# g1n0st/drake

Hardware: AMD Instinct MI355X
Metric: mpm_substeps_per_sec_1M_particles (higher is better)
Workload: dtype f32

## Files before the change

### drake_amd/csrc/mpm_step.h

```cpp
#pragma once
#include "mpm_device.h"

namespace mpm {

MPM_DEV bool gated_out(const DP& p) {
    return ((p.gated & 1) && p.ctl->need_rebuild) || ((p.gated & 2) && (p.ctl->error & ERR_SLABS)) ||
           ((p.gated & 4) && (int)(p.ctl->watch_hit - p.watch_base) >= 0);
}

template <int FM>
__global__ __launch_bounds__(256) void k_fem(DP p, float dt) {
#define MPM_FEM_MATERIAL_SETUP
#define MPM_FEM_M p.M
#define MPM_FEM_VOLW p.dist.on ? S.q[0][i].w : f2.w
#include "mpm_fem_face.inc"
#undef MPM_FEM_MATERIAL_SETUP
#undef MPM_FEM_M
#undef MPM_FEM_VOLW
}

struct ClothMat {
    float mu, lambda, gamma, K, cF, rho, pad0, pad1;
};
constexpr int FACE_CLOTH_SHIFT = 12;
MPM_DEV Material cloth_material(const Material& engine, const ClothMat* mats, const float4& f3) {
    const ClothMat t = mats[(unsigned)__float_as_int(f3.x) >> FACE_CLOTH_SHIFT];
    Material m = engine;
    m.mu = t.mu; m.lambda = t.lambda; m.gamma = t.gamma; m.K = t.K; m.cF = t.cF; m.density = t.rho;
    return m;
}

template <int FM>
__global__ __launch_bounds__(256) void k_fem_mat(DP p, float dt, const ClothMat* mats) {
#define MPM_FEM_MATERIAL_SETUP const Material M = cloth_material(p.M, mats, f3);
#define MPM_FEM_M M
#define MPM_FEM_VOLW f2.w * M.density
#include "mpm_fem_face.inc"
#undef MPM_FEM_MATERIAL_SETUP
#undef MPM_FEM_M
#undef MPM_FEM_VOLW
}

MPM_DEV bool vertex_force_vf(const DP& p, int k, float& f0, float& f1, float& f2) {
    const float* e0 = p.VF + vf_entry((unsigned)k, 0) * 3;
    float3 g[8];
#pragma unroll
    for (int j = 0; j < 8; ++j) g[j] = *reinterpret_cast<const float3*>(e0 + (size_t)j * VF_CHUNK * 3);
    f0 = f1 = f2 = 0.f;
#pragma unroll
    for (int j = 0; j < 8; ++j) {
        f0 += -g[j].x;
        f1 += -g[j].y;
        f2 += -g[j].z;
    }
    return __float_as_uint(g[0].x) != VF_MARK;
}

MPM_DEV void vertex_force_csr(const DP& p, const PSet& S, int k, float& f0, float& f1, float& f2) {
    const int s = p.Nf + k;
    f0 = f1 = f2 = 0.f;
    const int vo = S.pid[s] - p.NfG;
    for (int e = p.adj_off[vo]; e < p.adj_off[vo + 1]; ++e) {
        const int fc = p.adj_fc[e];
        const int fs = p.imap[fc >> 2];
        const float3 g = fs >= 0 ? p.G3[(size_t)fs * 3 + (fc & 3)]
                                 : make_float3(S.q[0][s].w > 0.f ? __int_as_float(0x7FC00000) : 0.f, 0.f, 0.f);
        f0 += -g.x;
        f1 += -g.y;
        f2 += -g.z;
    }
}

MPM_DEV void vertex_force_value(const DP& p, const PSet& S, int k, float& f0, float& f1, float& f2) {
    if (!vertex_force_vf(p, k, f0, f1, f2)) vertex_force_csr(p, S, k, f0, f1, f2);
}
MPM_DEV void vertex_force(const DP& p, const PSet& S, int k) {
    float f0, f1, f2;
    vertex_force_value(p, S, k, f0, f1, f2);
    const int s = p.Nf + k;
    p.f[0][s] = f0;
    p.f[1][s] = f1;
    p.f[2][s] = f2;
}

__global__ __launch_bounds__(256) void k_vforce(DP p) {
    if (gated_out(p)) return;
    const unsigned nva = (unsigned)p.ctl->nva;
    const unsigned chunk = xcd_chunk_active(blockIdx.x, nva);
    const int k = (int)(chunk * 256 + threadIdx.x);
    if (chunk == 0xFFFFFFFFu || k >= (int)nva) return;
    vertex_force(p, p.set[p.ctl->cur], k);
}

typedef float f32x4 __attribute__((ext_vector_type(4)));
typedef float f32x2 __attribute__((ext_vector_type(2)));

constexpr int STG = 16, STG_FX = 13;

MPM_DEV void lds_add_fixed(long long* a, float q, unsigned& worst) {
    const float aq = fabsf(q);
    const float h = floorf(aq * 0x1p-32f);
    const unsigned lo = (unsigned)rintf(fmaf(-h, 0x1p32f, aq));
    const unsigned long long mag = ((unsigned long long)(unsigned)h << 32) | lo;
    const unsigned long long fx = q < 0.f ? 0ull - mag : mag;
    __hip_atomic_fetch_add(reinterpret_cast<unsigned long long*>(a), fx, __ATOMIC_RELAXED,
                           __HIP_MEMORY_SCOPE_WORKGROUP);
    worst = max(worst, __float_as_uint(aq));
}

MPM_DEV void bspline_coeff(int a, bool on, float& c0, float& c1, float& c2) {
    c0 = a == 0 ? 1.125f : (a == 1 ? -.25f : .125f);
    c1 = a == 0 ? -1.5f : (a == 1 ? 2.f : -.5f);
    c2 = a == 1 ? -1.f : .5f;
    if (!on) c0 = c1 = c2 = 0.f;
}

struct Stencil {
    int rx, ry, rz;
    float fx[3];
    float wx[3], wy[3], wz[3];
    unsigned out_bits;
};

MPM_DEV Stencil make_stencil(const DP& p, float x, float y, float z, int ox, int oy, int oz) {
    Stencil s;
    const uint32_t hi = (uint32_t)((1 << p.bits) - 3);
    const uint32_t bx = min(base_cell(x, p.dxinv), hi), by = min(base_cell(y, p.dxinv), hi),
                   bz = min(base_cell(z, p.dxinv), hi);
    s.fx[0] = x * p.dxinv - (float)bx;
    s.fx[1] = y * p.dxinv - (float)by;
    s.fx[2] = z * p.dxinv - (float)bz;
    bspline3(s.fx[0], s.wx);
    bspline3(s.fx[1], s.wy);
    bspline3(s.fx[2], s.wz);
    int rx = (int)bx - ox, ry = (int)by - oy, rz = (int)bz - oz;
    const int hi_h = TILE_W - 3;
    static_assert(((TILE_W - 3) & (TILE_W - 2)) == 0, "rx | ry | rz <= hi_h is only equivalent to all three in range for hi_h = 2^k - 1");
    s.out_bits = (unsigned)(rx | ry | rz);
    rx = min(max(rx, 0), hi_h);
    ry = min(max(ry, 0), hi_h);
    rz = min(max(rz, 0), hi_h);
    s.rx = rx; s.ry = ry; s.rz = rz;
    return s;
}

MPM_DEV unsigned tile_reach_mask(int rx, int ry, int rz) {
    static_assert(FREE_ZONE == 2, "the packed tables below are for a free zone of 2 cells");
    const int ix = rx >> 1, iy = ry >> 1, iz = rz >> 1;
    const unsigned long long Z = 0x926D924DBull, Y = 0xE07E0703Full;
    const unsigned m9 = (unsigned)((Z >> (9 * iz)) & (Y >> (9 * iy))) & 0x1FFu;
    const unsigned rep = m9 * 0x40201u;
    const int lo = (ix + 1) >> 1, hi = (ix >> 1) + 1;
    const unsigned xexp = ((1u << (9 * (hi + 1))) - 1u) ^ ((1u << (9 * lo)) - 1u);
    return rep & xexp;
}

constexpr int P2G_WAVES = 8, P2G_THREADS = 64 * P2G_WAVES;
MPM_DEV f32x4 p2g_mfma(float y, float w, f32x4 acc) { return __builtin_amdgcn_mfma_f32_16x16x4f32(y, w, acc, 0, 0, 0); }
template <int FORCES, int EXACT>
__global__ __launch_bounds__(P2G_THREADS) __attribute__((amdgpu_waves_per_eu(P2G_WAVES / 2, P2G_WAVES / 2))) void k_p2g(DP p, float dt) {
    if (gated_out(p)) return;
    if (blockIdx.x == 0 && threadIdx.x < 2 && p.halo_hdr[threadIdx.x]) p.halo_hdr[threadIdx.x][0] = 0u;
    __shared__ long long tile[TILE_N * 4];
    __shared__ __attribute__((aligned(16))) float stage_all[P2G_WAVES][(64 + 8) * STG];
    __shared__ unsigned s_mask;
    static_assert(sizeof(long long) * TILE_N * 4 + sizeof(float) * P2G_WAVES * (64 + 8) * STG + 4 <= 81920,
                  "two workgroups per CU need <= 80 KB of LDS each");
    Ctl* ctl = p.ctl;
    const PSet& S = p.set[ctl->cur];
    const int tid = threadIdx.x, lane = tid & 63, wv = tid >> 6;
    const float gdt = p.M.gravity * dt;
    const float sdt = -dt * p.Dinv;
    float* stage = stage_all[wv];

    const int j16 = lane & 15, g4 = lane >> 4;
    float ax[2][3], ay[2][3], az[2][3];
#pragma unroll
    for (int t = 0; t < 2; ++t) {
        const int n = 16 * t + j16;
        const bool on = n < 27;
        bspline_coeff(n / 9, on, ax[t][0], ax[t][1], ax[t][2]);
        bspline_coeff((n / 3) % 3, true, ay[t][0], ay[t][1], ay[t][2]);
        bspline_coeff(n % 3, true, az[t][0], az[t][1], az[t][2]);
    }
    const f32x2 cx0 = {ax[0][0], ax[1][0]}, cx1 = {ax[0][1], ax[1][1]}, cx2 = {ax[0][2], ax[1][2]};
    const f32x2 cy0 = {ay[0][0], ay[1][0]}, cy1 = {ay[0][1], ay[1][1]}, cy2 = {ay[0][2], ay[1][2]};
    const f32x2 cz0 = {az[0][0], az[1][0]}, cz1 = {az[0][1], az[1][1]}, cz2 = {az[0][2], az[1][2]};
    float fac[2][4];
    int delta[2];
#pragma unroll
    for (int t = 0; t < 2; ++t) {
        const int n = 16 * t + j16;
        const int ni = n / 9, nj = (n / 3) % 3, nk = n % 3;
#pragma unroll
        for (int r = 0; r < 4; ++r) {
            fac[t][r] = n >= 27 ? 0.f : (r == 0 ? 1.f : (float)(r == 1 ? ni : (r == 2 ? nj : nk)));
            if (g4 == 3 && r != 0) fac[t][r] = 0.f;
        }
        delta[t] = n < 27 ? ((ni * TILE_W + nj) * TILE_W + nk) * 4 + g4 : -1;
    }
    {
        const float fscale = EXACT ? (float)(g4 == 3 ? p.fix_m : p.fix_p) : 1.f;
#pragma unroll
        for (int t = 0; t < 2; ++t)
#pragma unroll
            for (int r = 0; r < 4; ++r) fac[t][r] *= fscale;
    }
    const unsigned reach_of_lane = tile_reach_mask(2 * (lane >> 4), 2 * ((lane >> 2) & 3), 2 * (lane & 3));
    for (int k = lane; k < (64 + 8) * STG; k += 64) stage[k] = 0.f;

    const unsigned n_items = ctl->n_items;
    for (unsigned q = blockIdx.x; q < n_items; q += gridDim.x) {
        __syncthreads();
        const int4 fa = p.item_flat[2 * q], fb = p.item_flat[2 * q + 1];
        const unsigned item = (unsigned)fa.x;
        const unsigned long long tb0 = (diag_flags(p) & 4) ? __builtin_readcyclecounter() : 0ull;
        for (int n = tid; n < TILE_N * 4; n += P2G_THREADS) tile[n] = 0;
        if (tid == 0) s_mask = 0;
        int bx, by, bz;
        block_coords((uint32_t)fa.z, bx, by, bz);
        const int ox = bx * 4 - FREE_ZONE, oy = by * 4 - FREE_ZONE, oz = bz * 4 - FREE_ZONE;
        const int4 rg = make_int4(fb.x, fb.y, fb.z, 0);
        const int nfb = rg.y - rg.x;
        const int ngroups = fa.w;
        const int4* groups = p.home_groups + fb.w;
        struct Raw {
            float x[3], v[3], vol, C[9];
            float ta[3], tb[3], frc[3];
            bool act, is_face;
        };
        auto force_of = [&](unsigned ii, float* f) {
            const float* fbase = p.f[0] + ii;
#pragma unroll
            for (int d = 0; d < 3; ++d) f[d] = fbase[(size_t)d * p.f_stride];
        };
        auto desc_of = [&](int g) { return groups[min(g, ngroups - 1)]; };
        int4 gd_next = make_int4(0, 0, 0, 0);
        auto load_raw = [&](int4 gr) {
            Raw r;
            const int gf = gr.y - gr.x, gn = gf + (gr.w - gr.z);
            r.act = lane < gn;
            r.is_face = lane < gf;
            const unsigned any_slot = (unsigned)(nfb ? rg.x : rg.z);
            const unsigned ii = r.act ? (unsigned)(r.is_face ? gr.x + lane : gr.z + (lane - gf)) : any_slot;
            const float4* qb = S.q[0] + ii;
            const float4 q0 = qb[0], q1 = qb[p.q_stride], q2 = qb[2 * (size_t)p.q_stride], q3 = qb[3 * (size_t)p.q_stride];
            r.x[0] = q0.x; r.x[1] = q0.y; r.x[2] = q0.z; r.vol = q0.w;
            r.v[0] = q1.x; r.v[1] = q1.y; r.v[2] = q1.z;
            unpack_C(q1, q2, q3, r.C);
            {
                const unsigned fi = r.is_face ? ii : (unsigned)(nfb ? rg.x : 0), vi = r.is_face ? any_slot : ii;
                const float3 a = p.ta[fi];
                const float3 b = *reinterpret_cast<const float3*>(&S.fq[0][fi]);
                r.ta[0] = a.x; r.ta[1] = a.y; r.ta[2] = a.z; r.tb[0] = b.x; r.tb[1] = b.y; r.tb[2] = b.z;
                const bool vert = r.act && !r.is_face;
                if (FORCES == 1) {
                    vertex_force_vf(p, vert ? (int)ii - p.Nf : 0, r.frc[0], r.frc[1], r.frc[2]);
                } else {
                    force_of(vi, r.frc);
                }
                if (FORCES != 0 && vert && !p.lean_g2p) {
                    p.f[0][ii] = r.frc[0]; p.f[1][ii] = r.frc[1]; p.f[2][ii] = r.frc[2];
                }
            }
            return r;
        };
        Raw cur;
        __syncthreads();
        unsigned mymask = 0;
        bool halo_bad = false;
        unsigned out_worst = 0, fix_worst = 0;
        if (wv < ngroups) gd_next = desc_of(wv);
        const bool prof = (diag_flags(p) & 4) != 0 && wv == 0;
        unsigned long long tq[3] = {0, 0, 0}, pc[8] = {0, 0, 0, 0, 0, 0, 0, 0};
        if (prof && lane == 0) atomicAdd(&p.dbgbuf[14], (unsigned long long)__builtin_readcyclecounter() - tb0);
        for (int g = wv; g < ngroups; g += P2G_WAVES) {
            if (prof) tq[0] = __builtin_readcyclecounter();
            cur = load_raw(gd_next);
            gd_next = desc_of(g + P2G_WAVES);
            const bool act = cur.act, is_face = cur.is_face;
            const Stencil st = make_stencil(p, cur.x[0], cur.x[1], cur.x[2], ox, oy, oz);
            const bool own = cur.vol > 0.f;
            const float m = own ? cur.vol * p.M.density : 0.f;
            float Y[16];
            {
                float B[9];
                float fext[3] = {0.f, 0.f, 0.f};
#pragma unroll
                for (int r = 0; r < 9; ++r) B[r] = cur.C[r] * m;
                if (is_face) {
#pragma unroll
                    for (int r = 0; r < 3; ++r)
#pragma unroll
                        for (int c = 0; c < 3; ++c) B[r * 3 + c] = fmaf(sdt, cur.ta[r] * cur.tb[c], B[r * 3 + c]);
                } else {
#pragma unroll
                    for (int r = 0; r < 3; ++r) fext[r] = cur.frc[r] * dt;
                }
#pragma unroll
                for (int r = 0; r < 3; ++r) {
                    float qq = r == p.M.gravity_axis ? fmaf(cur.v[r], m, m * gdt) : cur.v[r] * m;
                    qq += fext[r];
                    const float dot = fmaf(B[r * 3 + 2], st.fx[2], fmaf(B[r * 3], st.fx[0], B[r * 3 + 1] * st.fx[1]));
                    qq = fmaf(-p.dx, dot, qq);
                    Y[r * 4 + 0] = qq;
                    Y[r * 4 + 1] = B[r * 3 + 0] * p.dx;
                    Y[r * 4 + 2] = B[r * 3 + 1] * p.dx;
                    Y[r * 4 + 3] = B[r * 3 + 2] * p.dx;
                }
                Y[12] = m; Y[13] = 0.f; Y[14] = 0.f; Y[15] = 0.f;
                if (p.dist.on && !own) {
#pragma unroll
                    for (int k = 0; k < 12; ++k) Y[k] = 0.f;
                }
            }
            out_worst = max(out_worst, act ? st.out_bits : 0u);
            if (p.dist.on && act && own) {
                const int gx = ox + st.rx;
                halo_bad |= gx < p.dist.own_lo - p.dist.zone_cells || gx + 2 >= p.dist.own_hi + p.dist.zone_cells;
            }
            if (diag_flags(p) & 2) {
                float acc = 0.f;
#pragma unroll
                for (int k = 0; k < 16; ++k) acc += Y[k];
                if (acc == 1.2345e30f) tile[0] = (long long)acc;
                continue;
            }
            const int key = (st.rx * 8 + st.ry) * 8 + st.rz;
            const unsigned long long actmask = __ballot(act);
            int pos = 0;
            {
                unsigned long long todo = actmask;
                int base = 0;
                while (todo) {
                    const int lk = __builtin_amdgcn_readlane(key, __builtin_ctzll(todo));
                    const bool mine = key == lk;
                    const unsigned long long same = __ballot(mine) & todo;
                    const int rank = (int)__builtin_amdgcn_mbcnt_hi((unsigned)(same >> 32), __builtin_amdgcn_mbcnt_lo((unsigned)same, (unsigned)base));
                    if (mine) pos = rank;
                    base += (int)__popcll(same);
                    todo &= ~same;
                }
            }
            if (act) {
                float4* sp = reinterpret_cast<float4*>(stage + pos * STG);
                sp[0] = make_float4(Y[0], Y[1], Y[2], Y[3]);
                sp[1] = make_float4(Y[4], Y[5], Y[6], Y[7]);
                sp[2] = make_float4(Y[8], Y[9], Y[10], Y[11]);
                sp[3] = make_float4(Y[12], st.fx[0], st.fx[1], st.fx[2]);
            }
            __builtin_amdgcn_fence(__ATOMIC_RELEASE, "wavefront");
            __builtin_amdgcn_wave_barrier();
            __builtin_amdgcn_fence(__ATOMIC_ACQUIRE, "wavefront");
            if (diag_flags(p) & 1) continue;
            unsigned long long todo = actmask;
            int s0 = 0;
            float nfx, nfy, nfz, ny;
            {
                const float* sn = stage + g4 * STG;
                nfx = sn[STG_FX]; nfy = sn[STG_FX + 1]; nfz = sn[STG_FX + 2]; ny = sn[j16];
            }
            if (prof) tq[1] = __builtin_readcyclecounter();
            __builtin_amdgcn_s_setprio(2);
            while (todo) {
                const int ckey = __builtin_amdgcn_readlane(key, __builtin_ctzll(todo));
                const unsigned long long same = __ballot(key == ckey) & todo;
                todo &= ~same;
                const int s1 = s0 + (int)__popcll(same);
                f32x4 acc0 = {0.f, 0.f, 0.f, 0.f}, acc1 = {0.f, 0.f, 0.f, 0.f};
                if (prof) { pc[4] += 1; pc[5] += (unsigned)((s1 - s0 + 3) >> 2); tq[2] = __builtin_readcyclecounter(); }
                auto step = [&](int s, bool first_step, bool last_step) {
                    const float fx = nfx, fy = nfy, fz = nfz;
                    float y = ny;
                    {
                        const float* sn = stage + (s + 4 + g4) * STG;
                        nfx = sn[STG_FX]; nfy = sn[STG_FX + 1]; nfz = sn[STG_FX + 2]; ny = sn[j16];
                    }
                    const f32x2 fx2 = {fx, fx}, fy2 = {fy, fy}, fz2 = {fz, fz};
                    const f32x2 w01 = __builtin_elementwise_fma(__builtin_elementwise_fma(cx2, fx2, cx1), fx2, cx0) *
                                      __builtin_elementwise_fma(__builtin_elementwise_fma(cy2, fy2, cy1), fy2, cy0) *
                                      __builtin_elementwise_fma(__builtin_elementwise_fma(cz2, fz2, cz1), fz2, cz0);
                    if (last_step && !(g4 < s1 - s)) y = 0.f;
                    if (first_step) {
                        const f32x4 zero = {0.f, 0.f, 0.f, 0.f};
                        acc0 = p2g_mfma(y, w01.x, zero);
                        acc1 = p2g_mfma(y, w01.y, zero);
                    } else {
                        acc0 = p2g_mfma(y, w01.x, acc0);
                        acc1 = p2g_mfma(y, w01.y, acc1);
                    }
                };
                const int last = s0 + ((s1 - s0 - 1) & ~3);
                if (last == s0) {
                    step(s0, true, true);
                } else {
                    step(s0, true, false);
                    for (int s = s0 + 4; s < last; s += 4) step(s, false, false);
                    step(last, false, true);
                }
                if (((s1 - s0) & 3) != 0) {
                    const float* sn = stage + (s1 + g4) * STG;
                    nfx = sn[STG_FX]; nfy = sn[STG_FX + 1]; nfz = sn[STG_FX + 2]; ny = sn[j16];
                }
                if (prof) { asm volatile("" :: "v"(acc0), "v"(acc1)); const unsigned long long tm = __builtin_readcyclecounter(); pc[2] += tm - tq[2]; tq[2] = tm; }
                s0 = s1;
                const int crx = ckey >> 6, cry = (ckey >> 3) & 7, crz = ckey & 7;
                mymask |= (unsigned)__builtin_amdgcn_readlane((int)reach_of_lane, ((ckey >> 3) & 0x30) | ((ckey >> 2) & 0xC) | ((ckey >> 1) & 3));
                long long* tb = tile + ((crx * TILE_W + cry) * TILE_W + crz) * 4;
#pragma unroll
                for (int t = 0; t < 2; ++t) {
                    const f32x4 a = t ? acc1 : acc0;
                    float val;
                    {
#pragma clang fp contract(off)
                        const float x0 = a[0] * fac[t][0], x1 = a[1] * fac[t][1], x2 = a[2] * fac[t][2], x3 = a[3] * fac[t][3];
                        val = (x0 + x1) + (x2 + x3);
                    }
                    if (delta[t] >= 0 && !(diag_flags(p) & 16)) {
                        if (EXACT) lds_add_fixed(tb + delta[t], val, fix_worst);
                        else __hip_atomic_fetch_add(reinterpret_cast<double*>(tb + delta[t]), (double)val, __ATOMIC_RELAXED, __HIP_MEMORY_SCOPE_WORKGROUP);
                    }
                }
                if (prof) pc[3] += __builtin_readcyclecounter() - tq[2];
            }
            if (prof) {
                const unsigned long long te = __builtin_readcyclecounter();
                pc[0] += tq[1] - tq[0];
                pc[1] += te - tq[1];
                pc[6] += 1;
            }
            __builtin_amdgcn_s_setprio(0);
            __builtin_amdgcn_fence(__ATOMIC_RELEASE, "wavefront");
            __builtin_amdgcn_wave_barrier();
        }
        if (prof) pc[7] = __builtin_readcyclecounter() - tb0;
        if (prof && lane == 0)
            for (int q = 0; q < 8; ++q) atomicAdd(&p.dbgbuf[q], pc[q]);
        if (mymask && lane == 0) atomicOr(&s_mask, mymask);
        if (__ballot(out_worst > (unsigned)(TILE_W - 3)) && lane == 0) atomicOr(&ctl->error, ERR_DRIFT);
        if (EXACT && __ballot(fix_worst >= __float_as_uint(0x1p62f)) && lane == 0) atomicOr(&ctl->error, ERR_RANGE);
        if (p.dist.on && __ballot(halo_bad) && lane == 0) atomicOr(&ctl->error, ERR_HALO);
        __syncthreads();
        if (prof && lane == 0) atomicAdd(&p.dbgbuf[15], (unsigned long long)__builtin_readcyclecounter() - tb0 - pc[7]);
        float4* out = p.slab + (size_t)item * TILE_N;
        bool not_finite = false;
        for (int n = tid; n < TILE_N; n += P2G_THREADS) {
            const long long* q = tile + n * 4;
            float4 o;
            if (EXACT) {
                o = make_float4((float)((double)q[0] * p.unfix_p), (float)((double)q[1] * p.unfix_p),
                                (float)((double)q[2] * p.unfix_p), (float)((double)q[3] * p.unfix_m));
            } else {
                const double* d = reinterpret_cast<const double*>(q);
                o = make_float4((float)d[0], (float)d[1], (float)d[2], (float)d[3]);
                not_finite |= !(fabsf(o.x) + fabsf(o.y) + fabsf(o.z) + fabsf(o.w) < __int_as_float(0x7F800000));
            }
            out[n] = o;
        }
        if (!EXACT && __ballot(not_finite) && lane == 0) atomicOr(&ctl->error, ERR_RANGE);
        if (tid == 0) p.slab_mask[item] = s_mask;
        if ((diag_flags(p) & 4) && tid == 0) {
            atomicAdd(&p.dbgbuf[12], (unsigned long long)__builtin_readcyclecounter() - tb0);
            atomicAdd(&p.dbgbuf[13], 1ull);
        }
    }
}

struct GridCollider {
    int shape;
    int mode;
    float p[3], n[3], radius, v[3], friction;
};
constexpr int MAX_GRID_COLLIDERS = 16;
struct GridColliders {
    int n;
    GridCollider c[MAX_GRID_COLLIDERS];
};

constexpr int GRID_LIST = 160;
MPM_DEV int __reduce_max_sync_i32(int v) {
#pragma unroll
    for (int d = 32; d >= 1; d >>= 1) v = max(v, __shfl_xor(v, d));
    return v;
}

MPM_DEV size_t halo_ids_offset() { return 4; }
MPM_DEV size_t halo_data_offset(unsigned cap) { return ((size_t)(4 + cap) * 4 + 15) / 16; }
template <int MODE>
__global__ __launch_bounds__(256) void k_grid(DP p, GridColliders gc) {
    __shared__ int2 s_list[4][GRID_LIST];
    const Ctl* ctl = p.ctl;
    {
        const bool out = gated_out(p);
        if (blockIdx.x == 0 && threadIdx.x == 0) p.ctl->skip_this = out;
        if (out) return;
    }
    const unsigned n_active = ctl->n_active;
    const int tid = threadIdx.x;
    const int cell = tid & 63;
    const int cx = cell >> 4, cy = (cell >> 2) & 3, cz = cell & 3;
    if (MODE == 0 && blockIdx.x == 0 && tid < 2 && p.halo_hdr[tid]) p.halo_hdr[tid][0] = 0u;
    if (MODE == 2 && p.halo_pn > 0 && tid < 64 && blockIdx.x * 64u < p.halo_pcap) {
        for (int k = 0; k < p.halo_pn; ++k) {
            const uint32_t* buf = p.halo_pbuf[k];
            const unsigned n = min(buf[0], p.halo_pcap);
            for (unsigned e = blockIdx.x * 64u + (unsigned)tid; e < n; e += gridDim.x * 64u) {
                const uint32_t id = buf[halo_ids_offset() + e];
                if (id >= p.nblocks) {
                    atomicOr(&p.ctl->error, ERR_HALO);
                    continue;
                }
                if (p.lut_act[id] < 0) continue;
                int hx, hy, hz;
                block_coords(id, hx, hy, hz);
                if (hx < p.halo_plo[k] || hx > p.halo_phi[k]) atomicOr(&p.ctl->error, ERR_CAPACITY);
            }
        }
    }
    for (unsigned a = blockIdx.x * 4 + (tid >> 6); a < n_active; a += gridDim.x * 4) {
        if (MODE == 2 && p.halo_cls >= 0) {
            int hx, hy, hz;
            block_coords(p.act_block[a], hx, hy, hz);
            if (!halo_block_selected(p, hx)) continue;
        }
        const int* nbr = p.act_nbr_items + (size_t)a * 27;
        float4 s = make_float4(0.f, 0.f, 0.f, 0.f);
        if (MODE == 2) {
            s = p.gv[(size_t)a * 64 + cell];
            if (p.halo_pn > 0) {
                const uint32_t myid = p.act_block[a];
                int bx, by, bz;
                block_coords(myid, bx, by, bz);
                for (int k = 0; k < p.halo_pn; ++k) {
                    if (bx < p.halo_plo[k] || bx > p.halo_phi[k]) continue;
                    const uint32_t* buf = p.halo_pbuf[k];
                    const unsigned n = min(buf[0], p.halo_pcap);
                    int found = -1;
                    for (unsigned base = 0; base < n && found < 0; base += 64) {
                        const uint32_t id = base + (unsigned)cell < n ? buf[halo_ids_offset() + base + (unsigned)cell] : 0xFFFFFFFFu;
                        const unsigned long long m = __ballot(id == myid);
                        if (m) found = (int)base + __builtin_ctzll(m);
                    }
                    if (found >= 0) {
                        const float4 r = (reinterpret_cast<const float4*>(buf) + halo_data_offset(p.halo_pcap))[(size_t)found * 64 + cell];
                        s.x += r.x; s.y += r.y; s.z += r.z; s.w += r.w;
                    }
                }
            }
        }
        if (MODE != 2) {
            int2* list = s_list[tid >> 6];
            const int packed = cell < 27 ? nbr[cell] : -1;
            const int it0 = packed & 0xFFFFFF, ni = packed < 0 ? 0 : (packed >> 24);
            int cnt = 0;
            const int nimax = __reduce_max_sync_i32(ni);
            for (int k = 0; k < nimax; ++k) {
                const bool hit = k < ni && ((p.slab_mask[it0 + k] >> (26 - cell)) & 1u);
                const unsigned long long m = __ballot(hit);
                if (hit) {
                    const int at = cnt + (int)__popcll(m & ((1ull << cell) - 1ull));
                    if (at < GRID_LIST) list[at] = make_int2(it0 + k, cell);
                }
                cnt += (int)__popcll(m);
            }
            __builtin_amdgcn_fence(__ATOMIC_RELEASE, "wavefront");
            __builtin_amdgcn_wave_barrier();
            __builtin_amdgcn_fence(__ATOMIC_ACQUIRE, "wavefront");
            if (cnt > GRID_LIST) {
                if (cell == 0) atomicOr(&p.ctl->error, ERR_CAPACITY);
                cnt = GRID_LIST;
            }
#pragma unroll 4
            for (int e = 0; e < cnt; ++e) {
                const int2 en = list[e];
                const int it = en.x, o = en.y;
                const int tx = cx - 4 * (o / 9 - 1) + FREE_ZONE;
                const int ty = cy - 4 * ((o / 3) % 3 - 1) + FREE_ZONE;
                const int tz = cz - 4 * (o % 3 - 1) + FREE_ZONE;
                const bool in_tile = !(tx < 0 || ty < 0 || tz < 0 || tx >= TILE_W || ty >= TILE_W || tz >= TILE_W);
                const int node = in_tile ? (tx * TILE_W + ty) * TILE_W + tz : 0;
                const float4 t = p.slab[(size_t)it * TILE_N + node];
                s.x += in_tile ? t.x : 0.f; s.y += in_tile ? t.y : 0.f;
                s.z += in_tile ? t.z : 0.f; s.w += in_tile ? t.w : 0.f;
            }
            __builtin_amdgcn_wave_barrier();
        }
        const size_t gi = (size_t)a * 64 + cell;
        if (MODE == 0) {
            p.gv[gi] = s;
            if (p.halo_pn > 0) {
                int bx, by, bz;
                block_coords(p.act_block[a], bx, by, bz);
                for (int k = 0; k < p.halo_pn; ++k) {
                    if (bx < p.halo_plo[k] || bx > p.halo_phi[k]) continue;
                    const int nbx = bx + p.halo_pshift[k];
                    if (nbx < 0 || nbx >= p.nb) continue;
                    uint32_t* buf = p.halo_pbuf[k];
                    unsigned slot = 0;
                    if (cell == 0) slot = atomicAdd(p.halo_pcnt[k] ? p.halo_pcnt[k] : &buf[0], 1u);
                    slot = __builtin_amdgcn_readfirstlane(slot);
                    if (slot >= p.halo_pcap) {
                        if (cell == 0) atomicOr(&p.ctl->error, ERR_CAPACITY);
                        continue;
                    }
                    if (cell == 0) buf[halo_ids_offset() + slot] = block_id((uint32_t)nbx, (uint32_t)by, (uint32_t)bz);
                    (reinterpret_cast<float4*>(buf) + halo_data_offset(p.halo_pcap))[(size_t)slot * 64 + cell] = s;
                }
            }
            continue;
        }
        float4 vs = make_float4(0.f, 0.f, 0.f, 0.f);
        if (s.w > 0.f) {
            float v[3] = {s.x / s.w, s.y / s.w, s.z / s.w};
            int bx, by, bz;
            block_coords(p.act_block[a], bx, by, bz);
            const int gx = bx * 4 + cx, gy = by * 4 + cy, gz = bz * 4 + cz;
            const int N = 1 << p.bits, wl = p.M.wall;
            if (gx < wl && v[0] < 0.f) v[0] = 0.f;
            if (gx >= N - wl && v[0] > 0.f) v[0] = 0.f;
            if (gy < wl && v[1] < 0.f) v[1] = 0.f;
            if (gy >= N - wl && v[1] > 0.f) v[1] = 0.f;
            if (gz < wl && v[2] < 0.f) v[2] = 0.f;
            if (gz >= N - wl && v[2] > 0.f) v[2] = 0.f;
            if (gc.n > 0) {
                const float pos[3] = {((float)gx + .5f) * p.dx, ((float)gy + .5f) * p.dx, ((float)gz + .5f) * p.dx};
                for (int k = 0; k < gc.n; ++k) {
                    const GridCollider& cl = gc.c[k];
                    float n[3], dist;
                    if (cl.shape == 0) {
                        const float d0 = pos[0] - cl.p[0], d1 = pos[1] - cl.p[1], d2 = pos[2] - cl.p[2];
                        const float len = sqrtf(d0 * d0 + d1 * d1 + d2 * d2);
                        const float inv = 1.f / len;
                        n[0] = d0 * inv; n[1] = d1 * inv; n[2] = d2 * inv;
                        dist = len - cl.radius;
                    } else {
                        n[0] = cl.n[0]; n[1] = cl.n[1]; n[2] = cl.n[2];
                        dist = n[0] * (pos[0] - cl.p[0]) + n[1] * (pos[1] - cl.p[1]) + n[2] * (pos[2] - cl.p[2]);
                    }
                    if (!(dist < 0.f)) continue;
                    const float dv[3] = {cl.v[0] - v[0], cl.v[1] - v[1], cl.v[2] - v[2]};
                    const float dn = n[0] * dv[0] + n[1] * dv[1] + n[2] * dv[2];
                    if (cl.mode == 0) {
                        v[0] += dv[0]; v[1] += dv[1]; v[2] += dv[2];
                    } else if (cl.mode == 2 || dn > 0.f) {
                        const float fr = cl.friction;
                        const float frac = (float)((double)dn * (1.0 - (double)fr));
                        v[0] += dv[0] * fr + n[0] * frac;
                        v[1] += dv[1] * fr + n[1] * frac;
                        v[2] += dv[2] * fr + n[2] * frac;
                    }
                    break;
                }
            }
            s.x = v[0]; s.y = v[1]; s.z = v[2];
            vs = make_float4(v[0], v[1], v[2], 0.f);
        }
        p.gv[gi] = s;
        p.gvs[gi] = vs;
    }
}

constexpr int G2P_THREADS = 512, G2P_WAVES = 4;
constexpr int LOAD_TILE_NQ = (TILE_N + G2P_THREADS - 1) / G2P_THREADS;
MPM_DEV void load_tile(const DP& p, unsigned h, float4* tile, const float4* field, int nthreads, unsigned long long* stamps = nullptr) {
    const int* nbr = p.home_nbr_act + (size_t)h * 27;
    constexpr int NQ = LOAD_TILE_NQ;
    int a[NQ], cell[NQ];
#pragma unroll
    for (int q = 0; q < NQ; ++q) {
        const int n = min((int)threadIdx.x + q * nthreads, TILE_N - 1);
        const int tx = n / (TILE_W * TILE_W), ty = (n / TILE_W) % TILE_W, tz = n % TILE_W;
        const int qx = tx - FREE_ZONE + 4, qy = ty - FREE_ZONE + 4, qz = tz - FREE_ZONE + 4;
        a[q] = nbr[(qx >> 2) * 9 + (qy >> 2) * 3 + (qz >> 2)];
        cell[q] = ((qx & 3) << 4) + ((qy & 3) << 2) + (qz & 3);
    }
    if (MPM_DIAG && stamps) { asm volatile("s_waitcnt vmcnt(0)" ::: "memory"); stamps[0] = __builtin_readcyclecounter(); }
    float4 v[NQ];
#pragma unroll
    for (int q = 0; q < NQ; ++q) v[q] = field[(size_t)max(a[q], 0) * 64 + cell[q]];
    if (MPM_DIAG && stamps) { asm volatile("s_waitcnt vmcnt(0)" ::: "memory"); stamps[1] = __builtin_readcyclecounter(); }
#pragma unroll
    for (int q = 0; q < NQ; ++q) {
        const int n = (int)threadIdx.x + q * nthreads;
        if (n < TILE_N) tile[n] = a[q] >= 0 ? v[q] : make_float4(0.f, 0.f, 0.f, 0.f);
    }
}

MPM_DEV int g2p_particle(const DP& p, const PSet& S, const float4* tile, unsigned i, float x, float y, float z,
                            float vol, int ox, int oy, int oz, float dt) {
    const Stencil st = make_stencil(p, x, y, z, ox, oy, oz);
    int bits = 0;
    if (p.dist.on && vol < 0.f) {
        const int gx = ox + st.rx;
        if (gx < p.dist.own_lo - p.dist.zone_cells || gx + 2 >= p.dist.own_hi + p.dist.zone_cells) bits = 2;
    }
    float nv[3] = {0.f, 0.f, 0.f}, nC[9] = {0.f, 0.f, 0.f, 0.f, 0.f, 0.f, 0.f, 0.f, 0.f};
    const float4* base = tile + ((st.rx * TILE_W + st.ry) * TILE_W + st.rz);
    const float ez[3] = {st.wz[0] * (0.f - st.fx[2]), st.wz[1] * (1.f - st.fx[2]), st.wz[2] * (2.f - st.fx[2])};
    const float ey[3] = {st.wy[0] * (0.f - st.fx[1]), st.wy[1] * (1.f - st.fx[1]), st.wy[2] * (2.f - st.fx[1])};
    const f32x2 W0 = {st.wz[0], ez[0]}, W1 = {st.wz[1], ez[1]}, W2 = {st.wz[2], ez[2]};
    const f32x2 zero2 = {0.f, 0.f};
#pragma unroll
    for (int a = 0; a < 3; ++a) {
        f32x2 BB[3] = {zero2, zero2, zero2};
        float By[3] = {0.f, 0.f, 0.f};
#pragma unroll
        for (int b = 0; b < 3; ++b) {
            const float4* row = base + (a * TILE_W + b) * TILE_W;
            const float4 g0 = row[0], g1 = row[1], g2 = row[2];
            const float wb = st.wy[b], eb = ey[b];
            const f32x2 wb2 = {wb, wb};
            const float c0[3] = {g0.x, g0.y, g0.z}, c1[3] = {g1.x, g1.y, g1.z}, c2[3] = {g2.x, g2.y, g2.z};
#pragma unroll
            for (int r = 0; r < 3; ++r) {
                f32x2 AA;
                if (r == 2) {
                    const f32x2 z0 = {g0.z, g0.w}, z1 = {g1.z, g1.w}, z2 = {g2.z, g2.w};
                    asm("v_pk_mul_f32 %0, %1, %2 op_sel_hi:[1,0]\n\ts_nop 0\n\t"
                        "v_pk_fma_f32 %0, %3, %4, %0 op_sel_hi:[1,0,1]\n\ts_nop 0\n\t"
                        "v_pk_fma_f32 %0, %5, %6, %0 op_sel_hi:[1,0,1]"
                        : "=&v"(AA) : "v"(W0), "v"(z0), "v"(W1), "v"(z1), "v"(W2), "v"(z2));
                } else {
                    const f32x2 s0 = {c0[r], c0[r]}, s1 = {c1[r], c1[r]}, s2 = {c2[r], c2[r]};
                    AA = __builtin_elementwise_fma(W2, s2, __builtin_elementwise_fma(W1, s1, W0 * s0));
                }
                BB[r] = __builtin_elementwise_fma(wb2, AA, BB[r]);
                By[r] = fmaf(eb, AA.x, By[r]);
            }
        }
        const float wa = st.wx[a];
        const float ea = wa * ((float)a - st.fx[0]);
        const f32x2 wa2 = {wa, wa};
#pragma unroll
        for (int r = 0; r < 3; ++r) {
            f32x2 vc = {nv[r], nC[r * 3 + 2]};
            vc = __builtin_elementwise_fma(wa2, BB[r], vc);
            nv[r] = vc.x;
            nC[r * 3 + 2] = vc.y;
            nC[r * 3 + 0] = fmaf(ea, BB[r].x, nC[r * 3 + 0]);
            nC[r * 3 + 1] = fmaf(wa, By[r], nC[r * 3 + 1]);
        }
    }
    if (diag_flags(p) & 256) {
        if (nv[0] + nC[0] + nC[4] + nC[8] == 1.2345e30f) S.q[1][i].x = nv[0];
        return 0;
    }
    const float sc = 4.f * p.dxinv;
    const float ca = (p.M.V + 1.f) * .5f, cb = (p.M.V - 1.f) * .5f;
    float Cn[9];
#pragma unroll
    for (int r = 0; r < 3; ++r)
#pragma unroll
        for (int c = 0; c < 3; ++c) Cn[r * 3 + c] = fmaf(ca, sc * nC[r * 3 + c], cb * (sc * nC[c * 3 + r]));
    const float xn = x + nv[0] * dt, yn = y + nv[1] * dt, zn = z + nv[2] * dt;
    const bool is_face = i < (unsigned)p.Nf;
    const bool full = !(p.lean_g2p && is_face);
    S.q[2][i] = make_float4(Cn[0], Cn[1], Cn[2], Cn[3]);
    S.q[3][i] = make_float4(Cn[4], Cn[5], Cn[6], Cn[7]);
    if (full) {
        S.q[0][i] = make_float4(xn, yn, zn, vol);
        S.q[1][i] = make_float4(nv[0], nv[1], nv[2], Cn[8]);
    }
    if (is_face) S.c8[i] = Cn[8];
    const float guard = .125f, top = (float)(TILE_W - 2) - guard;
    const float tx = xn * p.dxinv - .5f - (float)ox, ty = yn * p.dxinv - .5f - (float)oy,
                tz = zn * p.dxinv - .5f - (float)oz;
    return bits | (int)!(tx >= guard && tx < top && ty >= guard && ty < top && tz >= guard && tz < top);
}

__global__ __launch_bounds__(G2P_THREADS) __attribute__((amdgpu_waves_per_eu(G2P_WAVES, G2P_WAVES))) void k_g2p(DP p, float dt) {
    __shared__ float4 tile[TILE_N];
    const Ctl* ctl = p.ctl;
    if (p.gated && ctl->skip_this) {
        if (blockIdx.x == 0 && threadIdx.x == 0) atomicAdd(&p.ctl->skipped, 1u);
        return;
    }
    if (blockIdx.x == 0 && threadIdx.x == 0) p.ctl->time_since_resort += dt;
    const PSet& S = p.set[ctl->cur];
    const unsigned n_items = ctl->n_items;
    for (unsigned q = blockIdx.x; q < n_items; q += gridDim.x) {
        __syncthreads();
        const int4 fa = p.item_flat[2 * q];
        const unsigned h = (unsigned)fa.y;
        if (p.halo_cls >= 0) {
            int hx, hy, hz;
            block_coords((uint32_t)fa.z, hx, hy, hz);
            if (!halo_item_selected(p, hx)) continue;
        }
        const bool prof = (diag_flags(p) & 4) != 0 || ((diag_flags(p) & 4096) != 0 && (blockIdx.x & 63u) == 5u && threadIdx.x < 64);
        unsigned long long t0 = 0, t1 = 0;
        if (prof) t0 = __builtin_readcyclecounter();
        const int4 rg = p.item_rng[q];
        const int nfb = rg.y - rg.x, total = nfb + (rg.w - rg.z);
        auto slot_of = [&](int u) { return (unsigned)(u < nfb ? rg.x + u : rg.z + (u - nfb)); };
        int u = (int)threadIdx.x;
        int left = 0;
        unsigned i = slot_of(u < total ? u : 0);
        float4 pq = S.q[0][i];
        unsigned long long ts[2] = {0, 0};
        load_tile(p, h, tile, p.gv, G2P_THREADS, prof ? ts : nullptr);
        __syncthreads();
        if (prof) t1 = __builtin_readcyclecounter();
        if (prof && (threadIdx.x & 63) == 0 && (diag_flags(p) & 4096)) {
            atomicAdd(&p.dbgbuf[12], ts[0] - t0);
            atomicAdd(&p.dbgbuf[13], ts[1] - ts[0]);
        }
        int bx, by, bz;
        block_coords((uint32_t)fa.z, bx, by, bz);
        const int ox = bx * 4 - FREE_ZONE, oy = by * 4 - FREE_ZONE, oz = bz * 4 - FREE_ZONE;
#pragma unroll 1
        for (; u < total; u += G2P_THREADS) {
            const unsigned ci = i;
            const float4 c = pq;
            const int un = u + G2P_THREADS;
            if (un < total) {
                i = slot_of(un);
                pq = S.q[0][i];
            }
            left |= g2p_particle(p, S, tile, ci, c.x, c.y, c.z, c.w, ox, oy, oz, dt);
        }
        if (__ballot(left & 1) && (threadIdx.x & 63) == 0) p.ctl->need_rebuild = 1;
        if (p.dist.on && __ballot(left & 2) && (threadIdx.x & 63) == 0) atomicOr(&p.ctl->error, ERR_HALO);
        if (prof && (threadIdx.x & 63) == 0) {
            const unsigned long long t2 = __builtin_readcyclecounter();
            atomicAdd(&p.dbgbuf[8], t1 - t0);
            atomicAdd(&p.dbgbuf[9], t2 - t1);
            atomicAdd(&p.dbgbuf[10], (unsigned long long)((total + G2P_THREADS - 1) / G2P_THREADS));
            atomicAdd(&p.dbgbuf[11], 1ull);
        }
    }
}


struct HaloZones {
    int lo[2], hi[2], shift[2];
    uint32_t* buf[2];
};
__global__ __launch_bounds__(256) void k_halo_pack2(DP p, HaloZones z, unsigned cap) {
    const int k = blockIdx.y;
    uint32_t* buf = z.buf[k];
    const int bx_lo = z.lo[k], bx_hi = z.hi[k], shift_bx = z.shift[k];
    const unsigned n_active = p.ctl->n_active;
    float4* data = reinterpret_cast<float4*>(buf) + halo_data_offset(cap);
    for (unsigned a = blockIdx.x * 4 + (threadIdx.x >> 6); a < n_active; a += gridDim.x * 4) {
        int bx, by, bz;
        block_coords(p.act_block[a], bx, by, bz);
        if (bx < bx_lo || bx > bx_hi) continue;
        const int nbx = bx + shift_bx;
        if (nbx < 0 || nbx >= p.nb) continue;
        unsigned slot = 0;
        if ((threadIdx.x & 63) == 0) slot = atomicAdd(&buf[0], 1u);
        slot = __builtin_amdgcn_readfirstlane(slot);
        if (slot >= cap) {
            if ((threadIdx.x & 63) == 0) atomicOr(&p.ctl->error, ERR_CAPACITY);
            continue;
        }
        if ((threadIdx.x & 63) == 0) buf[halo_ids_offset() + slot] = block_id((uint32_t)nbx, (uint32_t)by, (uint32_t)bz);
        data[(size_t)slot * 64 + (threadIdx.x & 63)] = p.gv[(size_t)a * 64 + (threadIdx.x & 63)];
    }
}
struct HaloBufs {
    const uint32_t* buf[2];
};

__global__ void k_halo_signal(uint32_t* flag_a, uint32_t* flag_b, uint32_t seq, const uint32_t* cnt_a, uint32_t* hdr_a,
                              const uint32_t* cnt_b, uint32_t* hdr_b, unsigned cap) {
    if (threadIdx.x != 0 || blockIdx.x != 0) return;
    if (hdr_a) __hip_atomic_store(hdr_a, min(*cnt_a, cap), __ATOMIC_RELAXED, __HIP_MEMORY_SCOPE_SYSTEM);
    if (hdr_b) __hip_atomic_store(hdr_b, min(*cnt_b, cap), __ATOMIC_RELAXED, __HIP_MEMORY_SCOPE_SYSTEM);
    __threadfence_system();
    asm volatile("s_waitcnt vmcnt(0)" ::: "memory");
    if (flag_a) __hip_atomic_store(flag_a, seq, __ATOMIC_RELEASE, __HIP_MEMORY_SCOPE_SYSTEM);
    if (flag_b) __hip_atomic_store(flag_b, seq, __ATOMIC_RELEASE, __HIP_MEMORY_SCOPE_SYSTEM);
}
__global__ void k_halo_wait(const uint32_t* flag_a, const uint32_t* flag_b, uint32_t seq, unsigned long long timeout_ticks, Ctl* ctl) {
    if (threadIdx.x != 0 || blockIdx.x != 0) return;
    const unsigned long long t0 = wall_clock64();
    while (true) {
        const bool a = !flag_a || (int)(__hip_atomic_load(flag_a, __ATOMIC_ACQUIRE, __HIP_MEMORY_SCOPE_SYSTEM) - seq) >= 0;
        const bool b = !flag_b || (int)(__hip_atomic_load(flag_b, __ATOMIC_ACQUIRE, __HIP_MEMORY_SCOPE_SYSTEM) - seq) >= 0;
        if (a && b) return;
        if (wall_clock64() - t0 > timeout_ticks) {
            atomicOr(&ctl->error, ERR_HALO);
            return;
        }
        __builtin_amdgcn_s_sleep(20);
    }
}
__global__ __launch_bounds__(256) void k_halo_add2(DP p, HaloBufs b, unsigned cap) {
    const uint32_t* buf = b.buf[blockIdx.y];
    const unsigned n = min(buf[0], cap);
    const float4* data = reinterpret_cast<const float4*>(buf) + halo_data_offset(cap);
    for (unsigned e = blockIdx.x * 4 + (threadIdx.x >> 6); e < n; e += gridDim.x * 4) {
        const uint32_t id = buf[halo_ids_offset() + e];
        if (id >= p.nblocks) continue;
        const int a = p.lut_act[id];
        if (a < 0) continue;
        if (p.halo_nz > 0) {
            int hx, hy, hz;
            block_coords(id, hx, hy, hz);
            if (!in_halo_zone(p, hx)) {
                if ((threadIdx.x & 63) == 0) atomicOr(&p.ctl->error, ERR_CAPACITY);
                continue;
            }
        }
        const size_t g = (size_t)a * 64 + (threadIdx.x & 63);
        const float4 r = data[(size_t)e * 64 + (threadIdx.x & 63)];
        float4 q = p.gv[g];
        q.x += r.x; q.y += r.y; q.z += r.z; q.w += r.w;
        p.gv[g] = q;
    }
}

}
```

Baseline: 9907.

## Precompute per-particle xy B-spline weight products in LDS staging for P2G MFMA loop

Moves the x/y quadratic B-spline evaluation out of the inner MFMA loop. Each particle now writes its nine px*py products into a wider staging row, and the inner step only evaluates the z polynomial before multiplying. The stage row layout changes to 23 floats, and the node-to-lane mapping is remapped so each lane reads one xy product per accumulator. The variable-length step loop is fully unrolled with a goto-based dispatch and fixed-offset prefetch loads. This cuts per-step VALU work and address arithmetic, at the cost of more LDS stores per particle and a wider, non-16-aligned stride that may cause bank conflicts.

```diff
diff --git a/drake_amd/csrc/mpm_step.h b/drake_amd/csrc/mpm_step.h
--- a/drake_amd/csrc/mpm_step.h
+++ b/drake_amd/csrc/mpm_step.h
@@ -95,7 +95,8 @@
 typedef float f32x4 __attribute__((ext_vector_type(4)));
 typedef float f32x2 __attribute__((ext_vector_type(2)));
 
-constexpr int STG = 16, STG_FX = 13;
+constexpr int STG = 23, STG_PXY = 8, STG_FZ = 17, STG_ROWS = 67;
+MPM_DEV int stg_col(int c) { return c < 8 ? c : c + 10; }
 
 MPM_DEV void lds_add_fixed(long long* a, float q, unsigned& worst) {
     const float aq = fabsf(q);
@@ -162,9 +163,9 @@
     if (gated_out(p)) return;
     if (blockIdx.x == 0 && threadIdx.x < 2 && p.halo_hdr[threadIdx.x]) p.halo_hdr[threadIdx.x][0] = 0u;
     __shared__ long long tile[TILE_N * 4];
-    __shared__ __attribute__((aligned(16))) float stage_all[P2G_WAVES][(64 + 8) * STG];
+    __shared__ __attribute__((aligned(16))) float stage_all[P2G_WAVES][STG_ROWS * STG];
     __shared__ unsigned s_mask;
-    static_assert(sizeof(long long) * TILE_N * 4 + sizeof(float) * P2G_WAVES * (64 + 8) * STG + 4 <= 81920,
+    static_assert(sizeof(long long) * TILE_N * 4 + sizeof(float) * P2G_WAVES * STG_ROWS * STG + 4 <= 81920,
                   "two workgroups per CU need <= 80 KB of LDS each");
     Ctl* ctl = p.ctl;
     const PSet& S = p.set[ctl->cur];
@@ -174,30 +175,23 @@
     float* stage = stage_all[wv];
 
     const int j16 = lane & 15, g4 = lane >> 4;
-    float ax[2][3], ay[2][3], az[2][3];
-#pragma unroll
-    for (int t = 0; t < 2; ++t) {
-        const int n = 16 * t + j16;
-        const bool on = n < 27;
-        bspline_coeff(n / 9, on, ax[t][0], ax[t][1], ax[t][2]);
-        bspline_coeff((n / 3) % 3, true, ay[t][0], ay[t][1], ay[t][2]);
-        bspline_coeff(n % 3, true, az[t][0], az[t][1], az[t][2]);
-    }
-    const f32x2 cx0 = {ax[0][0], ax[1][0]}, cx1 = {ax[0][1], ax[1][1]}, cx2 = {ax[0][2], ax[1][2]};
-    const f32x2 cy0 = {ay[0][0], ay[1][0]}, cy1 = {ay[0][1], ay[1][1]}, cy2 = {ay[0][2], ay[1][2]};
-    const f32x2 cz0 = {az[0][0], az[1][0]}, cz1 = {az[0][1], az[1][1]}, cz2 = {az[0][2], az[1][2]};
+    const int node[2] = {j16 < 15 ? j16 : -1, j16 >= 3 && j16 < 15 ? j16 + 12 : -1};
+    float cz0, cz1, cz2;
+    bspline_coeff(j16 % 3, true, cz0, cz1, cz2);
+    const int ycol = j16 < 13 ? stg_col(j16) : 0;
+    const int xycol = STG_PXY + j16 / 3;
     float fac[2][4];
     int delta[2];
 #pragma unroll
     for (int t = 0; t < 2; ++t) {
-        const int n = 16 * t + j16;
+        const int n = node[t];
         const int ni = n / 9, nj = (n / 3) % 3, nk = n % 3;
 #pragma unroll
         for (int r = 0; r < 4; ++r) {
-            fac[t][r] = n >= 27 ? 0.f : (r == 0 ? 1.f : (float)(r == 1 ? ni : (r == 2 ? nj : nk)));
+            fac[t][r] = n < 0 ? 0.f : (r == 0 ? 1.f : (float)(r == 1 ? ni : (r == 2 ? nj : nk)));
             if (g4 == 3 && r != 0) fac[t][r] = 0.f;
         }
-        delta[t] = n < 27 ? ((ni * TILE_W + nj) * TILE_W + nk) * 4 + g4 : -1;
+        delta[t] = n >= 0 ? ((ni * TILE_W + nj) * TILE_W + nk) * 4 + g4 : -1;
     }
     {
         const float fscale = EXACT ? (float)(g4 == 3 ? p.fix_m : p.fix_p) : 1.f;
@@ -207,7 +201,7 @@
             for (int r = 0; r < 4; ++r) fac[t][r] *= fscale;
     }
     const unsigned reach_of_lane = tile_reach_mask(2 * (lane >> 4), 2 * ((lane >> 2) & 3), 2 * (lane & 3));
-    for (int k = lane; k < (64 + 8) * STG; k += 64) stage[k] = 0.f;
+    for (int k = lane; k < STG_ROWS * STG; k += 64) stage[k] = 0.f;
 
     const unsigned n_items = ctl->n_items;
     for (unsigned q = blockIdx.x; q < n_items; q += gridDim.x) {
@@ -343,11 +337,20 @@
                 }
             }
             if (act) {
-                float4* sp = reinterpret_cast<float4*>(stage + pos * STG);
-                sp[0] = make_float4(Y[0], Y[1], Y[2], Y[3]);
-                sp[1] = make_float4(Y[4], Y[5], Y[6], Y[7]);
-                sp[2] = make_float4(Y[8], Y[9], Y[10], Y[11]);
-                sp[3] = make_float4(Y[12], st.fx[0], st.fx[1], st.fx[2]);
+                float px[3], py[3];
+#pragma unroll
+                for (int a = 0; a < 3; ++a) {
+                    float c0, c1, c2;
+                    bspline_coeff(a, true, c0, c1, c2);
+                    px[a] = fmaf(fmaf(c2, st.fx[0], c1), st.fx[0], c0);
+                    py[a] = fmaf(fmaf(c2, st.fx[1], c1), st.fx[1], c0);
+                }
+                float* sp = stage + pos * STG;
+#pragma unroll
+                for (int c = 0; c < 13; ++c) sp[stg_col(c)] = Y[c];
+#pragma unroll
+                for (int a = 0; a < 9; ++a) sp[STG_PXY + a] = px[a / 3] * py[a % 3];
+                sp[STG_FZ] = st.fx[2];
             }
             __builtin_amdgcn_fence(__ATOMIC_RELEASE, "wavefront");
             __builtin_amdgcn_wave_barrier();
@@ -355,32 +358,33 @@
             if (diag_flags(p) & 1) continue;
             unsigned long long todo = actmask;
             int s0 = 0;
-            float nfx, nfy, nfz, ny;
-            {
-                const float* sn = stage + g4 * STG;
-                nfx = sn[STG_FX]; nfy = sn[STG_FX + 1]; nfz = sn[STG_FX + 2]; ny = sn[j16];
-            }
+            float ny, nfz;
+            f32x2 nxy;
+            const float *ry, *rxy, *rz;
+            auto load_ops = [&](int off) {
+                ny = ry[off]; nxy = f32x2{rxy[off], rxy[off + 4]}; nfz = rz[off];
+            };
+            auto cell_rows = [&](int s) {
+                const float* row = stage + (s + g4) * STG;
+                ry = row + ycol; rxy = row + xycol; rz = row + STG_FZ;
+                load_ops(0);
+            };
+            cell_rows(0);
             if (prof) tq[1] = __builtin_readcyclecounter();
             __builtin_amdgcn_s_setprio(2);
             while (todo) {
                 const int ckey = __builtin_amdgcn_readlane(key, __builtin_ctzll(todo));
                 const unsigned long long same = __ballot(key == ckey) & todo;
                 todo &= ~same;
-                const int s1 = s0 + (int)__popcll(same);
+                const int s1 = s0 + __builtin_popcount((unsigned)same) + __builtin_popcount((unsigned)(same >> 32));
+                const int nsteps = (s1 - s0 + 3) >> 2;
                 f32x4 acc0 = {0.f, 0.f, 0.f, 0.f}, acc1 = {0.f, 0.f, 0.f, 0.f};
-                if (prof) { pc[4] += 1; pc[5] += (unsigned)((s1 - s0 + 3) >> 2); tq[2] = __builtin_readcyclecounter(); }
-                auto step = [&](int s, bool first_step, bool last_step) {
-                    const float fx = nfx, fy = nfy, fz = nfz;
+                if (prof) { pc[4] += 1; pc[5] += (unsigned)nsteps; tq[2] = __builtin_readcyclecounter(); }
+                auto step = [&](int k, bool first_step, bool last_step) {
+                    const float pz = fmaf(fmaf(cz2, nfz, cz1), nfz, cz0);
+                    const f32x2 w01 = nxy * f32x2{pz, pz};
                     float y = ny;
-                    {
-                        const float* sn = stage + (s + 4 + g4) * STG;
-                        nfx = sn[STG_FX]; nfy = sn[STG_FX + 1]; nfz = sn[STG_FX + 2]; ny = sn[j16];
-                    }
-                    const f32x2 fx2 = {fx, fx}, fy2 = {fy, fy}, fz2 = {fz, fz};
-                    const f32x2 w01 = __builtin_elementwise_fma(__builtin_elementwise_fma(cx2, fx2, cx1), fx2, cx0) *
-                                      __builtin_elementwise_fma(__builtin_elementwise_fma(cy2, fy2, cy1), fy2, cy0) *
-                                      __builtin_elementwise_fma(__builtin_elementwise_fma(cz2, fz2, cz1), fz2, cz0);
-                    if (last_step && !(g4 < s1 - s)) y = 0.f;
+                    if (last_step && !(g4 < s1 - s0 - 4 * k)) y = 0.f;
                     if (first_step) {
                         const f32x4 zero = {0.f, 0.f, 0.f, 0.f};
                         acc0 = p2g_mfma(y, w01.x, zero);
@@ -389,19 +393,21 @@
                         acc0 = p2g_mfma(y, w01.x, acc0);
                         acc1 = p2g_mfma(y, w01.y, acc1);
                     }
+                    if (!last_step) load_ops(4 * (k + 1) * STG);
                 };
-                const int last = s0 + ((s1 - s0 - 1) & ~3);
-                if (last == s0) {
-                    step(s0, true, true);
+                if (nsteps == 1) {
+                    step(0, true, true);
                 } else {
-                    step(s0, true, false);
-                    for (int s = s0 + 4; s < last; s += 4) step(s, false, false);
-                    step(last, false, true);
-                }
-                if (((s1 - s0) & 3) != 0) {
-                    const float* sn = stage + (s1 + g4) * STG;
-                    nfx = sn[STG_FX]; nfy = sn[STG_FX + 1]; nfz = sn[STG_FX + 2]; ny = sn[j16];
-                }
+                    step(0, true, false);
+#define MPM_P2G_MIDDLE(k) if (nsteps - 1 == k) goto last_step; step(k, false, false);
+                    MPM_P2G_MIDDLE(1) MPM_P2G_MIDDLE(2) MPM_P2G_MIDDLE(3) MPM_P2G_MIDDLE(4) MPM_P2G_MIDDLE(5)
+                    MPM_P2G_MIDDLE(6) MPM_P2G_MIDDLE(7) MPM_P2G_MIDDLE(8) MPM_P2G_MIDDLE(9) MPM_P2G_MIDDLE(10)
+                    MPM_P2G_MIDDLE(11) MPM_P2G_MIDDLE(12) MPM_P2G_MIDDLE(13) MPM_P2G_MIDDLE(14)
+#undef MPM_P2G_MIDDLE
+                last_step:
+                    step(nsteps - 1, false, true);
+                }
+                cell_rows(min(s1, 63));
                 if (prof) { asm volatile("" :: "v"(acc0), "v"(acc1)); const unsigned long long tm = __builtin_readcyclecounter(); pc[2] += tm - tq[2]; tq[2] = tm; }
                 s0 = s1;
                 const int crx = ckey >> 6, cry = (ckey >> 3) & 7, crz = ckey & 7;
```

Measured after the change: 10110 (median of 6 runs). +2.0%, better.
